# Kelvin-ywc/LPI

Measured on AMD Instinct MI355X. Metric: image-text pairs/sec fwd+bwd (ViT-B/16, bs256/GPU), higher is better.
Workload: dtype bf16; 1 GPU; BASELINE.json configs[2]: ViT-B/16 dual encoder bs=256/GPU prompt_depth=3 r=4 P=16, fwd+bwd incl. DecomposedPrompt grads + SGD step; global_batch=256, image=224x224, towers=lock step, GEMMs of one layer op grouped in one launch, parallelism=dp1, weights=synthetic (numpy Philox, CLIP-init scales), frozen

## Files before the change

include/lpi_hip.h:

```cpp
#ifndef LPI_HIP_H
#define LPI_HIP_H

#include <stdint.h>

#ifdef __cplusplus
extern "C" {
#endif

#define LPI_F32 0
#define LPI_BF16 1
#define LPI_F16 2

#define LPI_F32X3 4

#define LPI_EINVAL (-22)
#define LPI_ENOSYS (-38)

#define LPI_EPI_NONE 0
#define LPI_EPI_QUICKGELU 1
#define LPI_EPI_DQUICKGELU 2
#define LPI_EPI_LN 3
#define LPI_EPI_LN_QUICKGELU 4
#define LPI_EPI_RES_ROWSTATS 5

// ... 102 lines not shown
    const void* q; int ldq;
    const void* qkv; int ldqkv;
    const int32_t* idx;
    void* ctx; int ldctx;
    float* lse;
    const void* dctx; int lddctx;
    void* dq; int lddq;
    void* dqkv; int lddqkv;
    int causal;
    int shared_rows;
    float* shared_dkv;
} lpi_attn_pooled_desc;
int lpi_attn_pooled_fwd_pair(int dtype, const lpi_attn_pooled_desc* d , void* stream);
int lpi_attn_pooled_bwd_pair(int dtype, const lpi_attn_pooled_desc* d , void* stream);
int lpi_attn_pooled_fwd_desc(int dtype, const lpi_attn_pooled_desc* d, void* stream);
int lpi_attn_pooled_bwd_desc(int dtype, const lpi_attn_pooled_desc* d, void* stream);

int lpi_spool_attn_supported(int L, int H, int d);
int lpi_spool_attn_fwd(int w_dtype, int B, int L, int H, const void* q, int ldq, const void* Wqkv, int ldw, const void* WqkvT, int ldwt, const float* bqkv, const void* x, int ldx,
                       const float* mean, const float* rstd, const float* gamma, const float* beta, float* scratch, float* lse, void* ctx, int ldctx, void* stream);
int lpi_spool_attn_bwd(int B, int L, int H, const void* Wqkv , int ldw, const void* WqkvT , int ldwt, const void* x, int ldx, const float* mean,
                       const float* rstd, const float* gamma, float* scratch, const float* lse, const void* dctx, int lddctx, void* dq, int lddq, void* dh, int lddh,
                       void* stream);

int lpi_txt_embed_fwd_shared(int x_dtype, int B, int L, const int32_t* row_start, int shared_rows , int P, int d, const int64_t* ids,
                             const float* tok_emb, const float* pos, const float* ctx , void* x0, float* out_mean,
                             float* out_rstd, void* stream);
int lpi_attn_fwd_shared(int dtype, int B, int L, const int32_t* row_start, int shared_rows, int H, const void* qkv, int ldqkv, void* ctx, int ldctx,
                        float* lse, void* stream);
int lpi_attn_bwd_shared(int dtype, int B, int L, const int32_t* row_start, int shared_rows, int rows_needed, int H, const void* qkv, int ldqkv,
                        const void* ctx, int ldctx, const void* dctx, int lddctx, const float* lse, float* delta, void* dqkv, int lddqkv,
                        float* shared_dkv, void* stream);
int lpi_shared_kv_reduce(int dtype, int B, int shared_rows, int H, const float* partial, void* dqkv, int lddqkv, int accumulate, void* stream);
int lpi_layernorm_bwd_rows_varlen(int dy_dtype, int cast_dtype, int x_dtype, int B, int L, const int32_t* row_start, int row0, int P, int d,
                                  const void* dy, int lddy, const void* x, int ldx, const float* gamma, const float* mean, const float* rstd,
                                  float* dx, int lddx, void* dx_cast, int ldcast, int accumulate, void* stream);
int lpi_gather_batch_rows_varlen(int dtype, int B, int L, const int32_t* row_start, int row0, int P, int cols, const void* src, int ld_src,
                                 void* dst, int ld_dst, void* stream);
int lpi_rows_sum_over_batch_varlen(int dtype, int B, int L, const int32_t* row_start, int row0, int P, int d, const void* dx, float* out,
                                   int accumulate, void* stream);
int lpi_prompt_add_varlen(int x_dtype, int B, int L, const int32_t* row_start, int P, int d, void* x, const float* prompt_l, long prompt_bstride,
                          float* out_mean, float* out_rstd, void* stream);
int lpi_txt_embed_fwd_varlen(int x_dtype, int B, int L, const int32_t* row_start, int P, int d, const int64_t* ids, const float* tok_emb,
                             const float* pos, const float* ctx, long ctx_bstride, void* x0, float* out_mean, float* out_rstd, void* stream);

int lpi_prompt_cp_fwd(int Lyr, int P, int D, int r, const float* d1, const float* d2, const float* d3,
// ... 196 lines not shown
```

lpi_amd/_lib.py:

```python
from __future__ import annotations

import ctypes
import os
from ctypes import c_float, c_int, c_long, c_uint64, c_void_p

_HERE = os.path.dirname(os.path.abspath(__file__))
LIB_PATH = os.environ.get("LPI_LIB") or os.path.join(_HERE, "csrc", "liblpi_hip.so")

F32, BF16, F16 = 0, 1, 2
MX8 = 3
GEMM_K_128, GEMM_K_256, GEMM_K_256_TAIL, GEMM_K_256X128, GEMM_K_ROWS = 0, 1, 2, 3, 4
GEMM_K_MX8 = 5
F32X3 = 4
GEMM_K_X3 = 6
GEMM_K_MX8_256 = 7
EPI_NONE, EPI_QUICKGELU, EPI_DQUICKGELU, EPI_LN, EPI_LN_QUICKGELU, EPI_RES_ROWSTATS = 0, 1, 2, 3, 4, 5


class LpiError(RuntimeError):
    pass


class GemmDesc(ctypes.Structure):
    _fields_ = [("M", c_int), ("N", c_int), ("K", c_int), ("A", c_void_p), ("lda", c_int), ("B", c_void_p), ("ldb", c_int),
# ... 22 lines not shown
    "lpi_gemm_nt_mx8": [_I, _I, _I, _I, _P, _I, _P, _I, _P, _I, _P, _I, _P, _I, _P, _I, _P, _P, _I, _I, _F, _P],
    "lpi_gemm_mx8_256_ok": [_I, _I, _I],
    "lpi_gemm_nt_mx8_256": [_I, _I, _I, _I, _P, _I, _P, _I, _P, _I, _P, _I, _P, _I, _P, _I, _P, _P, _I, _I, _F, _P],
    "lpi_mx8_quantize": [_I, _I, _I, _P, _I, _P, _I, _P, _I, _P],
    "lpi_layernorm_mx8_fwd": [_I, _I, _I, _P, _I, _P, _P, _P, _I, _P, _I, _P, _P, _P],
    "lpi_layernorm_fwd": [_I, _I, _I, _I, _P, _I, _P, _P, _P, _I, _P, _P, _P],
    "lpi_layernorm_bwd": [_I, _I, _I, _I, _I, _P, _I, _P, _I, _P, _P, _P, _P, _I, _P, _I, _I, _P],
    "lpi_layernorm_fwd_pair": [_I, _I, _P, _P],
    "lpi_layernorm_bwd_pair": [_I, _I, _I, _P, _P],
    "lpi_layernorm_bwd_rows": [_I, _I, _I, _I, _I, _I, _I, _I, _P, _I, _P, _I, _P, _P, _P, _P, _I, _P, _I, _I, _P],
    "lpi_gather_batch_rows": [_I, _I, _I, _I, _I, _I, _P, _I, _P, _I, _P],
    "lpi_attn_fwd": [_I, _I, _I, _I, _P, _I, _P, _I, _P, _I, _P],
    "lpi_attn_bwd": [_I, _I, _I, _I, _P, _I, _P, _I, _P, _I, _P, _P, _P, _I, _I, _P],
    "lpi_attn_pooled_fwd": [_I, _I, _I, _I, _P, _I, _P, _I, _P, _P, _I, _P, _I, _P],
    "lpi_attn_pooled_bwd": [_I, _I, _I, _I, _P, _I, _P, _I, _P, _P, _I, _P, _P, _I, _P, _I, _I, _P],
    "lpi_attn_fwd_varlen": [_I, _I, _I, _P, _I, _P, _I, _P, _I, _P, _I, _P],
    "lpi_attn_bwd_varlen": [_I, _I, _I, _P, _I, _P, _I, _P, _I, _P, _I, _P, _P, _P, _I, _I, _P],
    "lpi_attn_fwd_pair": [_I, _P, _P],
    "lpi_attn_bwd_layout": [_I, _I, _I, _I, _I, _P, _I, _P, _I, _P, _I, _P, _P, _P, _I, _P, _P],
    "lpi_attn_fwd_one": [_I, _P, _P],
    "lpi_spool_attn_supported": [_I, _I, _I],
    "lpi_spool_attn_fwd": [_I, _I, _I, _I, _P, _I, _P, _I, _P, _I, _P, _P, _I, _P, _P, _P, _P, _P, _P, _P, _I, _P],
    "lpi_spool_attn_bwd": [_I, _I, _I, _P, _I, _P, _I, _P, _I, _P, _P, _P, _P, _P, _P, _I, _P, _I, _P, _I, _P],
    "lpi_attn_bwd_prefix": [_I, _I, _I, _P, _I, _I, _P, _I, _P, _I, _P, _I, _P, _P, _P, _I, _I, _P],
    "lpi_attn_pooled_fwd_varlen": [_I, _I, _I, _P, _I, _P, _I, _P, _I, _P, _P, _I, _P, _I, _P],
    "lpi_attn_pooled_bwd_varlen": [_I, _I, _I, _P, _I, _P, _I, _P, _I, _P, _P, _I, _P, _P, _I, _P, _I, _I, _P],
    "lpi_layernorm_bwd_rows_varlen": [_I, _I, _I, _I, _I, _P, _I, _I, _I, _P, _I, _P, _I, _P, _P, _P, _P, _I, _P, _I, _I, _P],
    "lpi_gather_batch_rows_varlen": [_I, _I, _I, _P, _I, _I, _I, _P, _I, _P, _I, _P],
    "lpi_rows_sum_over_batch_varlen": [_I, _I, _I, _P, _I, _I, _I, _P, _P, _I, _P],
    "lpi_prompt_add_varlen": [_I, _I, _I, _P, _I, _I, _P, _P, _L, _P, _P, _P],
    "lpi_txt_embed_fwd_varlen": [_I, _I, _I, _P, _I, _I, _P, _P, _P, _P, _L, _P, _P, _P, _P],
    "lpi_scatter_add_rows": [_I, _I, _I, _I, _P, _I, _P, _P, _I, _P],
    "lpi_prompt_cp_fwd": [_I, _I, _I, _I, _P, _P, _P, _F, _P, _P],
    "lpi_prompt_cp_bwd": [_I, _I, _I, _I, _P, _P, _P, _F, _P, _P, _P, _P, _I, _P, _P],
    "lpi_align_loss_fwd_bwd": [_I, _I, _I, _I, _P, _P, _F, _F, _P, _P, _P, _P],
    "lpi_nt_bxent_fwd_bwd": [_I, _I, _I, _P, _P, _F, _F, _P, _P, _I, _P, _P],
    "lpi_patchify": [_I, _I, _I, _I, _P, _P, _I, _P],
    "lpi_patchify_u8": [_I, _I, _I, _I, _P, _P, _P, _I, _P],
    "lpi_vis_assemble_fwd": [_I, _I, _I, _I, _I, _P, _I, _P, _P, _P, _L, _P, _P, _P, _P, _P, _P, _P, _P],
    "lpi_vis_assemble_bwd": [_I, _I, _I, _I, _I, _P, _P, _L, _P, _P, _P, _P, _P],
    "lpi_txt_embed_fwd": [_I, _I, _I, _I, _I, _P, _P, _P, _P, _L, _P, _P, _P, _P],
    "lpi_rows_sum_over_batch": [_I, _I, _I, _I, _I, _I, _P, _P, _I, _P],
    "lpi_prompt_add": [_I, _I, _I, _I, _I, _P, _P, _L, _P, _P, _P],
    "lpi_pool_ln_fwd": [_I, _I, _I, _I, _I, _P, _P, _P, _P, _P, _I, _P, _P, _P],
    "lpi_pool_ln_bwd": [_I, _I, _I, _I, _P, _I, _P, _P, _P, _P, _P, _P, _P, _P],
    "lpi_gather_rows": [_I, _I, _I, _I, _P, _P, _P, _P],
# ... 42 lines not shown
    "lpi_host_gather": [_P, _P, _I, _L, _I],
    "lpi_host_gather_v": [_P, _P, _P, _I, _I],
    "lpi_image_resample_workspace": [_I, _I, _P, _P],
    "lpi_image_resample_u8": [_I, _I, _P, _P, _L, _P, _L, _P, _P],
    "lpi_image_resample_workspace_f": [_I, _I, _I, _P, _P],
    "lpi_image_resample_u8_f": [_I, _I, _I, _P, _P, _L, _P, _L, _P, _P],
    "lpi_jpeg_info": [_P, _L, _P],
    "lpi_jpeg_decode_workspace": [_I, _P, _P, _P],
    "lpi_jpeg_decode_u8": [_I, _P, _P, _P, _L, _P, _P, _L, _P, _P, _L, _P],
    "lpi_jpeg_info_x": [_I, _P, _L, _P],
    "lpi_jpeg_decode_workspace_x": [_I, _I, _P, _P, _P],
    "lpi_jpeg_decode_u8_x": [_I, _I, _P, _P, _P, _L, _P, _P, _L, _P, _P, _L, _P],
    "lpi_bpe_create": [_P, _L],
    "lpi_bpe_destroy": [_P],
    "lpi_interact_workspace_floats": [_I, _I, _I, _I],
    "lpi_interact_fwd": [_I, _I, _I, _I, _I, _I, _P, _I, _P, _I, _P, _P, _P, _P, _P, _P, _P, _P, _P, _P, _F, _F, _P, _I, _P, _I, _P, _P],
    "lpi_interact_bwd": [_I, _I, _I, _I, _I, _I, _P, _I, _P, _I, _P, _P, _P, _P, _P, _P, _P, _P, _P, _P, _F, _F, _P, _I, _P, _I, _P, _I, _P, _I,
                         _P, _P, _P],
    "lpi_bpe_encode": [_P, _P, _P, _I],
    "lpi_bpe_tokenize": [_P, _P, _I, _I, _I, _P],
}
_RESTYPES = {"lpi_launch_count": c_uint64, "lpi_search_workspace": c_long, "lpi_bpe_create": c_void_p, "lpi_bpe_destroy": None}

EXPECTED_ABI = 618
VARIANT_OFFSET = 1000000

_lib = None


def load() -> ctypes.CDLL:
    global _lib
    if _lib is not None:
        return _lib
    import torch
    if not os.path.exists(LIB_PATH):
        raise LpiError(
            f"{LIB_PATH} not found: the MI355X HIP extension is not built. Run "
            f"`python -c 'import __graft_entry__ as g; g.build()'` or lpi_amd/csrc/build.sh. "
            f"There is no CPU fallback for the product path.")
    lib = ctypes.CDLL(LIB_PATH)
    for name, argtypes in SIGNATURES.items():
        try:
            fn = getattr(lib, name)
        except AttributeError as e:
            raise LpiError(f"{LIB_PATH} does not export {name}") from e
        fn.argtypes = argtypes
        fn.restype = _RESTYPES.get(name, c_int)
# ... 204 lines not shown
```

lpi_amd/csrc/api.hip:

```cpp
#include <atomic>
#include "common.h"

static std::atomic<uint64_t> g_launches{0};

extern "C" void lpi_count_launch() { g_launches.fetch_add(1, std::memory_order_relaxed); }
extern "C" uint64_t lpi_launch_count(void) { return g_launches.load(std::memory_order_relaxed); }
#ifndef LPI_ABI_VERSION
#define LPI_ABI_VERSION 618
#endif
#ifdef LPI_VARIANT_BUILD
extern "C" int lpi_version(void) { return LPI_ABI_VERSION + 1000000; }
#else
extern "C" int lpi_version(void) { return LPI_ABI_VERSION; }
#endif

int lpi_cu_count() {
    static std::atomic<int> cache[64];
    int dev = 0;
    if (hipGetDevice(&dev) != hipSuccess || dev < 0 || dev >= 64) dev = 0;
    int n = cache[dev].load(std::memory_order_relaxed);
    if (n == 0) {
        int v = 0;
        if (hipDeviceGetAttribute(&v, hipDeviceAttributeMultiprocessorCount, dev) != hipSuccess || v <= 0) v = 256;
        cache[dev].store(v, std::memory_order_relaxed);
        n = v;
    }
    return n;
}

static thread_local int t_last_gemm_kernel = -1;
void lpi_note_gemm_kernel(int which) { t_last_gemm_kernel = which; }
// ... 15 lines not shown
```

lpi_amd/csrc/attn_stream.hip:

```cpp
#include "common.h"
#include "../../include/lpi_hip.h"

namespace {

constexpr int HD = 64;
constexpr int HS = 16;
constexpr int NT = 512;
typedef __attribute__((ext_vector_type(2))) float f32x2;
typedef __attribute__((ext_vector_type(2))) _Float16 f16x2;

__device__ __forceinline__ float wave_sum(float v) {
#pragma unroll
    for (int o = 32; o > 0; o >>= 1) v += __shfl_xor(v, o);
    return v;
}
__device__ __forceinline__ float wave_max(float v) {
#pragma unroll
    for (int o = 32; o > 0; o >>= 1) v = fmaxf(v, __shfl_xor(v, o));
    return v;
}


template <typename T>
__global__ __launch_bounds__(256) void headw_t_kernel(int B, int H, int d, const T* __restrict__ in, int ldin, const T* __restrict__ WT, int ldwt, int col0, float scale,
// ... 375 lines not shown
                    if (l < L) *reinterpret_cast<uint2*>(orow + (jt + u) * 16) = make_uint2(pack2_t<bf16_t>(acc[0], acc[1]), pack2_t<bf16_t>(acc[2], acc[3]));
                }
            }
        }
    }
    {
        constexpr int NJ = KS / 4;
        f32x4 acc[NJ];
#pragma unroll
        for (int t = 0; t < NJ; ++t) acc[t] = f32x4{0.f, 0.f, 0.f, 0.f};
        weighted_row_sums_mfma<NJ, NJ>(acc, A.x + row0 * A.ldx, A.ldx, L, Lp, d, wt, xt);
        const int h = lane & 15, g = lane >> 4;
        if (h < H) {
            const float zm = zmu[h];
#pragma unroll
            for (int t = 0; t < NJ; ++t) {
                const int j = 16 * (wave + 8 * t) + 4 * g;
                if (j < d) *reinterpret_cast<f32x4*>(A.dqt + ((size_t)b * H + h) * d + j) = *reinterpret_cast<const f32x4*>(A.gamma + j) * (acc[t] - zm);
            }
        }
    }
}

size_t spool_lds(int L, int d, bool bwd) {
    const size_t Lp = (size_t)((L + 15) & ~15), rb = (size_t)d * 2 + 16;
    const size_t Lp32 = (Lp + 31) & ~(size_t)31, wt = HS * Lp32 * 2, xt = 32 * ((size_t)d * 2 + XT_PAD);
    if (!bwd) return HS * rb + Lp * HS * 4 + 2 * Lp * 4 + 2 * HS * 4 + wt + xt;
    return std::max(std::max(2 * HS * rb, (size_t)d * W2B), xt) + 2 * Lp * HS * 4 + Lp * 64 + 2 * Lp * 4 + 3 * HS * 4 + wt;
}

bool spool_ok(int L, int H, int d) { return H >= 1 && H <= HS && d == HD * H && d % 32 == 0 && d <= 2 * NT && L >= 1 && L <= 288 && spool_lds(L, d, true) <= 160 * 1024; }

template <bool BWD>
int spool_launch(const SpoolArgs& A, hipStream_t s) {
    const int KS = A.d / 32, NH = (A.H + 3) & ~3;
    const size_t lds = spool_lds(A.L, A.d, BWD);
#define SP(K, N)                                                                                                                   \
    if (KS == K && NH == N) {                                                                                                      \
        static LdsOnce once;                                                                                                       \
        const void* fn = BWD ? (const void*)spool_bwd_kernel<K, N> : (const void*)spool_fwd_kernel<K, N>;                          \
        if (int e = lpi_ensure_lds(once, fn, 160 * 1024)) return e;                                                                \
        if (BWD) LPI_LAUNCH((spool_bwd_kernel<K, N>), dim3(A.B), dim3(NT), lds, s, A);                                              \
        else LPI_LAUNCH((spool_fwd_kernel<K, N>), dim3(A.B), dim3(NT), lds, s, A);                                                  \
        LPI_CHECK_LAST();                                                                                                          \
        return 0;                                                                                                                  \
    }
    SP(24, 12) SP(32, 16) SP(4, 4) SP(8, 4) SP(16, 8)
#undef SP
    return LPI_ENOSYS;
}

template <typename T>
int headw_t(int B, int H, int d, const void* in, int ldin, const void* WT, int ldwt, int col0, float scale, float* out, hipStream_t s) {
    LPI_LAUNCH((headw_t_kernel<T>), dim3(H, (B + 15) / 16), dim3(256), 0, s, B, H, d, (const T*)in, ldin, (const T*)WT, ldwt, col0, scale, out);
// ... 30 lines not shown
    return w_dtype == LPI_BF16 ? headw_n<bf16_t, bf16_t>(B, H, d, hbar, Wqkv, ldw, 2 * d, bqkv, 1.0f, ctx, ldctx, s)
                               : headw_n<f16_t, f16_t>(B, H, d, hbar, Wqkv, ldw, 2 * d, bqkv, 1.0f, ctx, ldctx, s);
}

extern "C" int lpi_spool_attn_bwd(int B, int L, int H, const void* Wqkv, int ldw, const void* WqkvT, int ldwt, const void* x, int ldx, const float* mean,
                                  const float* rstd, const float* gamma, float* scratch, const float* lse, const void* dctx, int lddctx, void* dq, int lddq, void* dh,
                                  int lddh, void* stream) {
    const int d = HD * H;
    if (!Wqkv || !WqkvT || !x || !mean || !rstd || !gamma || !scratch || !lse || !dctx || !dq || !dh || B <= 0) return LPI_EINVAL;
    if (!spool_ok(L, H, d) || ldw < d || ldwt < 3 * d || ldx < d || lddctx < d || lddq < d || lddh < d || ((ldx | ldw | ldwt | lddctx) & 7) || (lddh & 3) ||
        (((uintptr_t)x | (uintptr_t)Wqkv | (uintptr_t)WqkvT | (uintptr_t)dctx) & 15) || ((uintptr_t)dh & 7) ||
        (((uintptr_t)scratch | (uintptr_t)gamma) & 15))
        return LPI_EINVAL;
    hipStream_t s = (hipStream_t)stream;
    const size_t n = (size_t)B * H * d;
    float* qt = scratch;
    float* dhbar = scratch + 2 * n;
    float* dqt = scratch + 3 * n;
    if (int e = headw_t<bf16_t>(B, H, d, dctx, lddctx, WqkvT, ldwt, 2 * d, 1.0f, dhbar, s)) return e;
    SpoolArgs A{B, L, H, d, (const f16_t*)x, ldx, mean, rstd, gamma, nullptr, qt, nullptr, const_cast<float*>(lse), dhbar, (bf16_t*)dh, lddh, dqt};
    if (int e = spool_launch<true>(A, s)) return e;
    return headw_n<bf16_t, bf16_t>(B, H, d, dqt, Wqkv, ldw, d, nullptr, 0.125f, dq, lddq, s);
}
```

lpi_amd/engine.py:

```python
from __future__ import annotations

import math
from dataclasses import dataclass
from typing import Optional

import numpy as np
import torch

from . import _lib
from ._lib import BF16, EPI_DQUICKGELU, EPI_LN, EPI_LN_QUICKGELU, EPI_NONE, EPI_QUICKGELU, EPI_RES_ROWSTATS, F16, F32, F32X3, call
from .synth import ClipConfig

import ctypes
import os as _os

_DT = {"f32": F32, "fp32": F32, "float32": F32, "bf16": BF16, "bfloat16": BF16, "f16": F16, "fp16": F16, "float16": F16, "half": F16}


def _grad_dtype(dt: int) -> int:
    return F32 if dt == F32 else BF16
_TORCH_DT = {F32: torch.float32, BF16: torch.bfloat16, F16: torch.float16}


PIXEL_NORMS = {"imagenet": (None, None),
               "clip": ((0.48145466, 0.4578275, 0.40821073), (0.26862954, 0.26130258, 0.27577711))}


@dataclass(frozen=True)
class EngineOptions:
    residual_f16: bool = True
    ln_fold: int = 2
    rowstats: int = 2
    rowstat_guard: bool = True
    pooled_last: bool = True
    stream_pool: bool = True
    l0_prompt_rows: bool = True
    qkv_grouped: bool = False
    pixel_norm: object = "imagenet"
    mx8_forward: bool = False
    mx8_tile256: bool = True
    gemm_bf16x3: bool = False

    def __post_init__(self):
        if self.ln_fold not in (0, 1, 2) or self.rowstats not in (0, 1, 2):
            raise ValueError("ln_fold and rowstats are 0, 1 or 2")
        if not isinstance(self.pixel_norm, str):
            try:
                mean, std = self.pixel_norm
                pair = (tuple(float(v) for v in mean), tuple(float(v) for v in std))
            except (TypeError, ValueError):
                raise ValueError(f"pixel_norm is 'imagenet', 'clip' or a (mean, std) pair, not {self.pixel_norm!r}") from None
            if len(pair[0]) != 3 or len(pair[1]) != 3:
                raise ValueError("pixel_norm: a (mean, std) pair holds three values each")
            object.__setattr__(self, "pixel_norm", pair)
        elif self.pixel_norm not in PIXEL_NORMS:
            raise ValueError(f"pixel_norm is 'imagenet', 'clip' or a (mean, std) pair, not {self.pixel_norm!r}")

    def check_dtype(self, dtype: str):
# ... 476 lines not shown
        Lreal, L = L, max(L, cap or L)
        Mp = _pad(B * L, 256)
        Bp = _pad(B)
        T, TX, TG = _TORCH_DT[self.dt], _TORCH_DT[self.xdt], _TORCH_DT[self.gdt]
        TU = TG if self.dt == F16 else T
        dev = self.device
        z = lambda *s, dtype=torch.float32: torch.zeros(*s, dtype=dtype, device=dev)
        keep = nl if train else 1
        ws = {
            "B": B, "L": L, "Mp": Mp, "Lcap": L,
            "x": [z(Mp, d, dtype=TX) for _ in range(nl + 1 if train else 2)],
            "xmid": [z(Mp, d, dtype=TX) for _ in range(keep)],
            "qkv": [z(Mp, 3 * d, dtype=T) for _ in range(keep)],
            "ctx": [z(Mp, d, dtype=T) for _ in range(keep)],
            "lse": [z(B + 1, H, L) for _ in range(keep)],
            "u": [z(Mp, 4 * d, dtype=TU) for _ in range(keep)] if train else [None],
            "lnblk": [z(2, 3 * Mp + 4 * d) for _ in range(nl)],
            "h": z(Mp, d, dtype=T),
            "g": z(Mp, 4 * d, dtype=T),
            "rstat": z(2 * max(d // 128, 1), Mp),
            "Bp": Bp, "c_xmid": z(Bp, d), "c_h": z(Bp, d, dtype=T), "c_g": z(Bp, 4 * d, dtype=T),
            "c_u": z(Bp, 4 * d, dtype=TU) if train else None, "c_xout": z(Bp, d), "c_stat": z(2, Bp),
            "c_q": z(Bp, d, dtype=T), "c_ctx": z(Bp, d, dtype=T), "c_lse": z(B * H), "c_xin": z(Bp, d), "c_stat1": z(2, Bp),
            "sp_scratch": z(4 * B * H * d) if self._stream_pool_shape(L) else None, "sp_lse": z(B * H),
        }
        if train:
            ws.update({
                "dx": z(Mp, d) if self.dt == F32 else None,
                "dh": z(Mp, d, dtype=TG), "dctx": z(Mp, d, dtype=TG), "dqkv": z(Mp, 3 * d, dtype=TG),
                "delta": z(B + 1, H, L),
                "dxT": z(Mp, d, dtype=TG) if self.dt != F32 else None,
                "c_dx": z(Bp, d), "c_dxT": z(Bp, d, dtype=TG) if self.dt != F32 else None, "c_dh": z(Bp, d, dtype=TG),
                "c_dctx": z(Bp, d, dtype=TG), "c_dq": z(Bp, d, dtype=TG),
                "p_dqkv": z(_pad(B * 32, 256), 3 * d, dtype=TG), "p_dh": z(_pad(B * 32, 256), d, dtype=TG),
                "du": None, "c_du": None,
            })
        if train:
            ws["du"], ws["c_du"] = ws["g"].view(TG), ws["c_g"].view(TG)
        if self.mx8 and not train:
            u8 = lambda *s: torch.zeros(*s, dtype=torch.uint8, device=dev)
            ws["mx"] = {"h": u8(Mp, d), "hs": u8(Mp, d // 32), "ctx": u8(Mp, d), "ctxs": u8(Mp, d // 32), "g": u8(Mp, 4 * d), "gs": u8(Mp, 4 * d // 32)}
        ws["stat"] = [(b[0, :Mp], b[0, Mp:2 * Mp], b[1, :Mp], b[1, Mp:2 * Mp]) for b in ws["lnblk"]]
        ws["ln_ld"] = Mp
        for i, blk in enumerate(self.blocks):
            if "qkv_ln" in blk:
                c1 = blk["qkv_ln"].c1
                if i == nl - 1 and POOLED_LAST:
# ... 137 lines not shown
        dxT = ws["dxT"] if dt != F32 else dx
        P = prompts.shape[-2] if prompts is not None else 0
        pre = ws.get("pre", 0)
        Bq, Lq, rsq = (1, pre, None) if pre else (B, L, rs)
        self._check_depth(prompts, depth)
        for i in reversed(range(len(self.blocks))):
            blk = self.blocks[i]
            lt = "last" if i == len(self.blocks) - 1 else f"r{len(self.blocks) - 1 - i}"
            x_in, xmid, qkv, ctx, lse, u, st = ws["x"][i], ws["xmid"][i], ws["qkv"][i], ws["ctx"][i], ws["lse"][i], ws["u"][i], ws["stat"][i]
            if i == len(self.blocks) - 1 and not POOLED_LAST:
                call("lpi_zero", dxT, dxT.numel() * dxT.element_size(), s)
                call("lpi_scatter_rows", dt, B, Lx, d, ws["c_dx"], pidx, dx, None if dt == F32 else dxT, s)
            if i == len(self.blocks) - 1 and POOLED_LAST:
                Bp, cst = ws["Bp"], ws["c_stat"]
                c_dx = ws["c_dx"]
                c_dxT = ws["c_dxT"] if dt != F32 else c_dx
                yield GemmReq(f"{lt}.cdproj", mdt, c_dxT, blk["proj"].wt, ws["c_du"], Bp, 4 * d, d, epi=EPI_DQUICKGELU, aux=ws["c_u"], m_real=B)
                yield GemmReq(f"{lt}.cdfc", mdt, ws["c_du"], blk["fc"].wt, ws["c_dh"], Bp, d, 4 * d, m_real=B)
                yield RowReq(f"{lt}.cdln2", [_lib.row_job(_lib.ROWOP_LN_BWD, B=B, d=d, dt_a=dt, dt_b=dt, a=ws["c_dh"], ld_a=d, b=ws["c_xmid"], ld_b=d,
                                                          gamma=blk["ln_2.w"], mean_in=cst[0], rstd_in=cst[1], out=c_dx, out2=None if dt == F32 else c_dxT,
                                                          ld_c=d, flag=1)])
                wqt = blk["qkv"].wt
                yield GemmReq(f"{lt}.cdout", mdt, c_dxT, blk["out"].wt, ws["c_dctx"], Bp, d, d, m_real=B)
                if rs is None and not pre and ws.get("sp_scratch") is not None and self._stream_pool_shape(L):
                    yield SoloReq(f"{lt}.pdattn", lambda: call("lpi_spool_attn_bwd", B, L, H, blk["qkv_wb"], d, blk["qkv"].wt, 3 * d, x_in, d, st[0], st[1], blk["ln_1.w"],
                                                               ws["sp_scratch"], ws["sp_lse"], ws["c_dctx"], d, ws["c_dq"], d, dh, d, _stream()))
                    yield SoloReq(f"{lt}.dkv")
                else:
                    yield PoolAttnReq(f"{lt}.pdattn", adt, True, B=B, L=L, row_start=rs, H=H, q=ws["c_q"], ldq=d, qkv=qkv, ldqkv=3 * d, idx=pool_idx,
                                      dctx=ws["c_dctx"], lddctx=d, lse=ws["c_lse"], dq=ws["c_dq"], lddq=d, dqkv=dqkv, lddqkv=3 * d, causal=int(sp.causal),
                                      shared_rows=pre, shared_dkv=ws.get("shared_dkv") if pre else None)
                    yield GemmReq(f"{lt}.dkv", mdt, dqkv[:, d:], wqt[:, d:], dh, Mp, d, 2 * d, m_real=M)
                yield GemmReq(f"{lt}.cdq", mdt, ws["c_dq"], wqt[:, :d], ws["c_dh"], Bp, d, d, m_real=B)
                yield RowReq(f"{lt}.sadd1", [_lib.row_job(_lib.ROWOP_SCATTER_ADD, B=B, L=Lx, d=d, dt_a=dt, a=ws["c_dh"], ld_a=d, idx=pidx, out=dh, ld_c=d)])
                yield LnReq(f"{lt}.dln1", "bwd", (dt, dt, xdt), M, d, dh, d, x_in, d, blk["ln_1.w"], st[0], st[1], dx, d,
                            None if dt == F32 else dxT, d, 0)
                yield RowReq(f"{lt}.sadd2", [_lib.row_job(_lib.ROWOP_SCATTER_ADD, B=B, L=Lx, d=d, dt_a=dt, a=c_dxT, ld_a=d, idx=pidx, out=dxT, ld_c=d)])
                if prompts is not None and dprompts is not None and 0 < i < depth:
                    yield RowsSumReq(f"{lt}.psum", dt, Bq, Lq, rsq, 1, P, d, dxT, dprompts[i], acc)
                continue
            if not (i == len(self.blocks) - 1 and POOLED_LAST):
                du = ws["du"]
                yield GemmReq(f"{lt}.dproj", mdt, dxT, blk["proj"].wt, du, Mp, 4 * d, d, epi=EPI_DQUICKGELU, aux=u, m_real=M)
                yield GemmReq(f"{lt}.dfc", mdt, du, blk["fc"].wt, dh, Mp, d, 4 * d, m_real=M)
                yield LnReq(f"{lt}.dln2", "bwd", (dt, dt, xdt), M, d, dh, d, xmid, d, blk["ln_2.w"], st[2], st[3], dx, d,
                            None if dt == F32 else dxT, d, 1)
            yield GemmReq(f"{lt}.dout", mdt, dxT, blk["out"].wt, dctx, Mp, d, d, m_real=M)
            l0_rows = i == 0 and L0_PROMPT_ROWS and prompts is not None and 0 < P <= 32 and len(self.blocks) > 1
            if pre:
                call("lpi_attn_bwd_shared", adt, B, L, rs, pre, (1 + P) if l0_rows else L, H, qkv, 3 * d, ctx, d, dctx, d, lse, ws["delta"], dqkv, 3 * d,
                     ws["shared_dkv"], s)
            elif blk["grouped"]:
                hs_, vs_, chs_ = self.qkv_lay
                lay = (ctypes.c_int32 * 6)(hs_, vs_, hs_, vs_, chs_, chs_)
                call("lpi_attn_bwd_layout", adt, B, L, (1 + P) if l0_rows else L, H, qkv, 3 * d, ctx, d, dctx, d, lse, ws["delta"], dqkv, 3 * d,
                     ctypes.cast(lay, ctypes.c_void_p), s)
# ... 599 lines not shown
```

Before: 11710 pairs/s.

## Fuse LN1 backward into streaming pooled-attention backward for last layer

Adds a streaming pooled-attention backward kernel that computes the LayerNorm-1 backward for every non-pooled row in place and writes bf16 dx directly. Only the pooled row's dy goes to a small fp32 buffer. A tiny follow-up kernel finishes the LN backward for that pooled row, adding the cdq and residual contributions. This removes the full-size dh intermediate, the scatter-add and the separate M x d LayerNorm backward pass over all tokens. In exchange the fused kernel carries more LDS and register pressure, and it rounds dy to bf16 inside the kernel.

```diff
diff --git a/include/lpi_hip.h b/include/lpi_hip.h
--- a/include/lpi_hip.h
+++ b/include/lpi_hip.h
@@ -148,6 +148,11 @@
 int lpi_spool_attn_bwd(int B, int L, int H, const void* Wqkv , int ldw, const void* WqkvT , int ldwt, const void* x, int ldx, const float* mean,
                        const float* rstd, const float* gamma, float* scratch, const float* lse, const void* dctx, int lddctx, void* dq, int lddq, void* dh, int lddh,
                        void* stream);
+int lpi_spool_attn_bwd_ln1(int B, int L, int H, const void* Wqkv , int ldw, const void* WqkvT , int ldwt, const void* x, int ldx, const float* mean,
+                           const float* rstd, const float* gamma, const float* beta, float* scratch, const float* lse, const void* dctx, int lddctx, void* dq, int lddq,
+                           const int* pidx, void* dxs, int lddxs, float* dpool, void* stream);
+int lpi_spool_pool_rows(int B, int L, int d, const int* pidx, const float* dpool, const void* c_dh, int ldcdh, const void* c_dx, int ldcdx, const void* x, int ldx,
+                        const float* mean, const float* rstd, const float* gamma, void* dxs, int lddxs, void* stream);
 
 int lpi_txt_embed_fwd_shared(int x_dtype, int B, int L, const int32_t* row_start, int shared_rows , int P, int d, const int64_t* ids,
                              const float* tok_emb, const float* pos, const float* ctx , void* x0, float* out_mean,
diff --git a/lpi_amd/_lib.py b/lpi_amd/_lib.py
--- a/lpi_amd/_lib.py
+++ b/lpi_amd/_lib.py
@@ -68,6 +68,8 @@
     "lpi_spool_attn_supported": [_I, _I, _I],
     "lpi_spool_attn_fwd": [_I, _I, _I, _I, _P, _I, _P, _I, _P, _I, _P, _P, _I, _P, _P, _P, _P, _P, _P, _P, _I, _P],
     "lpi_spool_attn_bwd": [_I, _I, _I, _P, _I, _P, _I, _P, _I, _P, _P, _P, _P, _P, _P, _I, _P, _I, _P, _I, _P],
+    "lpi_spool_attn_bwd_ln1": [_I, _I, _I, _P, _I, _P, _I, _P, _I, _P, _P, _P, _P, _P, _P, _P, _I, _P, _I, _P, _P, _I, _P, _P],
+    "lpi_spool_pool_rows": [_I, _I, _I, _P, _P, _P, _I, _P, _I, _P, _I, _P, _P, _P, _P, _I, _P],
     "lpi_attn_bwd_prefix": [_I, _I, _I, _P, _I, _I, _P, _I, _P, _I, _P, _I, _P, _P, _P, _I, _I, _P],
     "lpi_attn_pooled_fwd_varlen": [_I, _I, _I, _P, _I, _P, _I, _P, _I, _P, _P, _I, _P, _I, _P],
     "lpi_attn_pooled_bwd_varlen": [_I, _I, _I, _P, _I, _P, _I, _P, _I, _P, _P, _I, _P, _P, _I, _P, _I, _I, _P],
@@ -156,7 +158,7 @@
 }
 _RESTYPES = {"lpi_launch_count": c_uint64, "lpi_search_workspace": c_long, "lpi_bpe_create": c_void_p, "lpi_bpe_destroy": None}
 
-EXPECTED_ABI = 618
+EXPECTED_ABI = 619
 VARIANT_OFFSET = 1000000
 
 _lib = None
diff --git a/lpi_amd/csrc/api.hip b/lpi_amd/csrc/api.hip
--- a/lpi_amd/csrc/api.hip
+++ b/lpi_amd/csrc/api.hip
@@ -6,7 +6,7 @@
 extern "C" void lpi_count_launch() { g_launches.fetch_add(1, std::memory_order_relaxed); }
 extern "C" uint64_t lpi_launch_count(void) { return g_launches.load(std::memory_order_relaxed); }
 #ifndef LPI_ABI_VERSION
-#define LPI_ABI_VERSION 618
+#define LPI_ABI_VERSION 619
 #endif
 #ifdef LPI_VARIANT_BUILD
 extern "C" int lpi_version(void) { return LPI_ABI_VERSION + 1000000; }
diff --git a/lpi_amd/csrc/attn_stream.hip b/lpi_amd/csrc/attn_stream.hip
--- a/lpi_amd/csrc/attn_stream.hip
+++ b/lpi_amd/csrc/attn_stream.hip
@@ -421,6 +421,329 @@
     }
 }
 
+struct Spool1Args {
+    int B, L, H, d;
+    const f16_t* x; int ldx;
+    const float* mean; const float* rstd;
+    const float* gamma; const float* beta;
+    const float* qt; const float* hbar; const float* lse; const float* dhbar;
+    float* dqt;
+    const int* pidx;
+    bf16_t* dxs; int lddxs;
+    float* dpool;
+};
+
+constexpr int PART_BYTES = 8 * 2 * 2 * 16 * 16 * 4;
+
+template <int KS>
+__global__ __launch_bounds__(NT) void spool_bwd1_kernel(Spool1Args A) {
+    static_assert(KS % 4 == 0, "d is a multiple of 128");
+    constexpr int NJ = KS / 4, NKW = (KS + 7) / 8;
+    extern __shared__ __attribute__((aligned(16))) char smem[];
+    const int b = blockIdx.x, tid = threadIdx.x, lane = tid & 63, wave = tid >> 6, g = lane >> 4, r16 = lane & 15;
+    constexpr int d = 32 * KS, rsx = d * 2 + XT_PAD, cpr = d / 8;
+    const int L = A.L, H = A.H, Lp32 = (L + 31) & ~31, rb = grow_bytes(d);
+    char* xt = smem;
+    char* img0 = smem;
+    char* img1 = smem + HS * rb;
+    float* part = reinterpret_cast<float*>(smem + 32 * rsx);
+    char* PD = reinterpret_cast<char*>(part) + PART_BYTES;
+    char* wt = PD + 32 * 64;
+    float* red = reinterpret_cast<float*>(wt + 2 * HS * 32 * 2);
+    float* gam = red + 8 * 32 * 2;
+    float* mu_l = gam + d;
+    float* rs_l = mu_l + Lp32;
+    float* cg = rs_l + Lp32;
+    float* cgd = cg + HS;
+    float* dl = cgd + HS;
+    float* lse_s = dl + HS;
+    float* zmu = lse_s + HS;
+    const size_t row0 = (size_t)b * L;
+    const float* qtb = A.qt + (size_t)b * H * d;
+    const float* dhb = A.dhbar + (size_t)b * H * d;
+    const float* hbb = A.hbar + (size_t)b * H * d;
+    const int pl = A.pidx ? min(max(A.pidx[b], 0), L - 1) : 0;
+    stage_row_stats(mu_l, rs_l, A.mean, A.rstd, row0, L, Lp32);
+    for (int j = tid; j < d; j += NT) gam[j] = A.gamma[j];
+    if (tid < HS) lse_s[tid] = tid < H ? A.lse[(size_t)b * H + tid] : 0.f;
+    for (int h = wave; h < HS; h += NT / 64) {
+        float s = 0.f;
+        if (h < H)
+            for (int j = lane; j < d; j += 64) {
+                const float gm = A.gamma[j], dv = dhb[(size_t)h * d + j];
+                s += (hbb[(size_t)h * d + j] - A.beta[j]) * (gm != 0.f ? (float)(f16_t)(gm * dv) / gm : dv);
+            }
+        s = wave_sum(s);
+        if (lane == 0) dl[h] = s;
+    }
+    Chunk w2[NJ];
+#pragma unroll
+    for (int t = 0; t < NJ; ++t) {
+        const int j = 16 * (wave * NJ + t) + r16, hb = (g & 1) * 8;
+        const float* src = (g < 2 ? dhb : qtb) + j;
+        float v[8];
+#pragma unroll
+        for (int q = 0; q < 8; ++q) v[q] = hb + q < H ? src[(size_t)(hb + q) * d] : 0.f;
+        w2[t].u = make_uint4(pack2_t<f16_t>(v[0], v[1]), pack2_t<f16_t>(v[2], v[3]), pack2_t<f16_t>(v[4], v[5]), pack2_t<f16_t>(v[6], v[7]));
+        __builtin_amdgcn_sched_barrier(0);
+    }
+    fill_gamma_image(img0, cg, qtb, A.gamma, H, d);
+    fill_gamma_image(img1, cgd, dhb, A.gamma, H, d);
+    Chunk ia[NKW], ib[NKW];
+#pragma unroll
+    for (int c = 0; c < NKW; ++c) {
+        const int ks = wave + 8 * c;
+        ia[c].u = ib[c].u = make_uint4(0, 0, 0, 0);
+        if (ks < KS) {
+            ia[c].u = *reinterpret_cast<const uint4*>(img0 + r16 * rb + (g + 4 * ks) * 16);
+            ib[c].u = *reinterpret_cast<const uint4*>(img1 + r16 * rb + (g + 4 * ks) * 16);
+        }
+    }
+    f32x4 accq[NJ];
+#pragma unroll
+    for (int t = 0; t < NJ; ++t) accq[t] = f32x4{0.f, 0.f, 0.f, 0.f};
+    float zm = 0.f, spd = 0.f, sw = 0.f;
+    const f16_t* xs = A.x + row0 * A.ldx;
+    uint4 stg[NJ];
+    auto load_tile = [&](int l0) {
+#pragma unroll
+        for (int u = 0; u < NJ; ++u) {
+            const int c = tid + u * NT;
+            stg[u] = make_uint4(0, 0, 0, 0);
+            if (c < 32 * cpr) stg[u] = *reinterpret_cast<const uint4*>(xs + (size_t)min(l0 + c / cpr, L - 1) * A.ldx + (c % cpr) * 8);
+        }
+    };
+    load_tile(0);
+    for (int l0 = 0; l0 < Lp32; l0 += 32) {
+        __syncthreads();
+#pragma unroll
+        for (int u = 0; u < NJ; ++u) {
+            const int c = tid + u * NT;
+            if (c < 32 * cpr) *reinterpret_cast<uint4*>(xt + (c / cpr) * rsx + (c % cpr) * 16) = stg[u];
+        }
+        __syncthreads();
+        if (l0 + 32 < Lp32) load_tile(l0 + 32);
+#pragma unroll
+        for (int hf = 0; hf < 2; ++hf) {
+            f32x4 a0 = f32x4{0.f, 0.f, 0.f, 0.f}, a1 = f32x4{0.f, 0.f, 0.f, 0.f};
+#pragma unroll
+            for (int c = 0; c < NKW; ++c) {
+                const int ks = wave + 8 * c;
+                Chunk xb;
+                xb.u = make_uint4(0, 0, 0, 0);
+                if (ks < KS) xb.u = *reinterpret_cast<const uint4*>(xt + (hf * 16 + r16) * rsx + (g + 4 * ks) * 16);
+                mma_chunk<f16_t>(a0, ia[c], xb);
+                mma_chunk<f16_t>(a1, ib[c], xb);
+            }
+            float* pp = part + ((wave * 2 + hf) * 2 * 16 + r16) * 16 + 4 * g;
+            *reinterpret_cast<f32x4*>(pp) = a0;
+            *reinterpret_cast<f32x4*>(pp + 16 * 16) = a1;
+        }
+        __syncthreads();
+        {
+            const int row = tid >> 4, h = tid & 15, l = l0 + row;
+            float a0 = 0.f, a1 = 0.f;
+#pragma unroll
+            for (int w = 0; w < 8; ++w) {
+                const float* pp = part + ((w * 2 + (row >> 4)) * 2 * 16 + (row & 15)) * 16 + h;
+                a0 += pp[0];
+                a1 += pp[16 * 16];
+            }
+            const float mu = mu_l[l], rs = rs_l[l];
+            float p = 0.f, ds = 0.f;
+            if (l < L && h < H) {
+                p = __expf(rs * (a0 - mu * cg[h]) - lse_s[h]);
+                const float dp = rs * (a1 - mu * cgd[h]), pw = (float)(f16_t)(p * rs) / rs;
+                ds = pw * (dp - dl[h]);
+                spd += pw * dp;
+                sw += pw;
+            }
+            const f16_t e = (f16_t)(ds * rs), e2 = (f16_t)(ds * rs - (float)e);
+            zm += ((float)e + (float)e2) * mu;
+            *reinterpret_cast<f16_t*>(PD + row * 64 + h * 2) = (f16_t)p;
+            *reinterpret_cast<f16_t*>(PD + row * 64 + 32 + h * 2) = (f16_t)ds;
+            *reinterpret_cast<f16_t*>(wt + (h * 32 + row) * 2) = e;
+            *reinterpret_cast<f16_t*>(wt + (HS * 32 + h * 32 + row) * 2) = e2;
+        }
+        __syncthreads();
+        auto g_tile = [&](int row, int t, const Chunk& pd, float mu, float rs, f32x4& dy, f32x4& gv, f32x4& xh) {
+            const int col = 16 * (wave * NJ + t) + 4 * g;
+            f32x4 acc = f32x4{0.f, 0.f, 0.f, 0.f};
+            mma_chunk<f16_t>(acc, w2[t], pd);
+            const f32x4 xv = Elem<f16_t>::ld4(reinterpret_cast<const f16_t*>(xt + row * rsx) + col);
+            const uint32_t r01 = pack2_t<bf16_t>(acc[0], acc[1]), r23 = pack2_t<bf16_t>(acc[2], acc[3]);
+            dy = f32x4{__uint_as_float(r01 << 16), __uint_as_float(r01 & 0xFFFF0000u), __uint_as_float(r23 << 16), __uint_as_float(r23 & 0xFFFF0000u)};
+            gv = dy * *reinterpret_cast<const f32x4*>(gam + col);
+            xh = (xv - mu) * rs;
+        };
+#pragma unroll
+        for (int hf = 0; hf < 2; ++hf) {
+            const int row = hf * 16 + r16;
+            Chunk pd;
+            pd.u = *reinterpret_cast<const uint4*>(PD + row * 64 + g * 16);
+            const float mu = mu_l[l0 + row], rs = rs_l[l0 + row];
+            float s1 = 0.f, s2 = 0.f;
+#pragma unroll
+            for (int t = 0; t < NJ; ++t) {
+                f32x4 dy, gv, xh;
+                g_tile(row, t, pd, mu, rs, dy, gv, xh);
+#pragma unroll
+                for (int i = 0; i < 4; ++i) {
+                    s1 += gv[i];
+                    s2 += gv[i] * xh[i];
+                }
+            }
+            s1 += __shfl_xor(s1, 16);
+            s2 += __shfl_xor(s2, 16);
+            s1 += __shfl_xor(s1, 32);
+            s2 += __shfl_xor(s2, 32);
+            if (g == 0) *reinterpret_cast<f32x2*>(red + (wave * 32 + row) * 2) = f32x2{s1, s2};
+        }
+        {
+            Chunk wb, wb2;
+            const uint2 lo = *reinterpret_cast<const uint2*>(wt + (r16 * 32 + 4 * g) * 2), hi = *reinterpret_cast<const uint2*>(wt + (r16 * 32 + 16 + 4 * g) * 2);
+            wb.u = make_uint4(lo.x, lo.y, hi.x, hi.y);
+            const uint2 lob = *reinterpret_cast<const uint2*>(wt + (HS * 32 + r16 * 32 + 4 * g) * 2), hib = *reinterpret_cast<const uint2*>(wt + (HS * 32 + r16 * 32 + 16 + 4 * g) * 2);
+            wb2.u = make_uint4(lob.x, lob.y, hib.x, hib.y);
+            const char* tp = xt + (4 * g + (r16 >> 2)) * rsx + (r16 & 3) * 8;
+#pragma unroll
+            for (int t = 0; t < NJ; ++t) {
+                const int jt = wave + 8 * t;
+                const short4s tlo = __builtin_amdgcn_ds_read_tr16_b64_v4i16((__attribute__((address_space(3))) short4s*)(tp + jt * 32));
+                const short4s thi = __builtin_amdgcn_ds_read_tr16_b64_v4i16((__attribute__((address_space(3))) short4s*)(tp + 16 * rsx + jt * 32));
+                const uint2 lo2 = __builtin_bit_cast(uint2, tlo), hi2 = __builtin_bit_cast(uint2, thi);
+                Chunk xa;
+                xa.u = make_uint4(lo2.x, lo2.y, hi2.x, hi2.y);
+                mma_chunk<f16_t>(accq[t], xa, wb);
+                mma_chunk<f16_t>(accq[t], xa, wb2);
+            }
+        }
+        __syncthreads();
+#pragma unroll
+        for (int hf = 0; hf < 2; ++hf) {
+            const int row = hf * 16 + r16, l = l0 + row;
+            float c1 = 0.f, c2 = 0.f;
+#pragma unroll
+            for (int w = 0; w < 8; ++w) {
+                const f32x2 q = *reinterpret_cast<const f32x2*>(red + (w * 32 + row) * 2);
+                c1 += q[0];
+                c2 += q[1];
+            }
+            c1 /= (float)d;
+            c2 /= (float)d;
+            const float mu = mu_l[l], rs = rs_l[l];
+            const bool pooled = l == pl;
+            Chunk pd;
+            pd.u = *reinterpret_cast<const uint4*>(PD + row * 64 + g * 16);
+            bf16_t* orow = A.dxs + (row0 + l) * A.lddxs + 4 * g;
+            float* prow = A.dpool + (size_t)b * d + 4 * g;
+#pragma unroll
+            for (int t = 0; t < NJ; ++t) {
+                f32x4 dy, gv, xh;
+                g_tile(row, t, pd, mu, rs, dy, gv, xh);
+                if (l < L) {
+                    if (pooled) {
+                        *reinterpret_cast<f32x4*>(prow + 16 * (wave * NJ + t)) = dy;
+                    } else {
+                        const f32x4 o = (gv - c1 - xh * c2) * rs;
+                        *reinterpret_cast<uint2*>(orow + 16 * (wave * NJ + t)) = make_uint2(pack2_t<bf16_t>(o[0], o[1]), pack2_t<bf16_t>(o[2], o[3]));
+                    }
+                }
+            }
+        }
+    }
+    __syncthreads();
+    part[tid] = zm;
+    part[NT + tid] = spd;
+    part[2 * NT + tid] = sw;
+    __syncthreads();
+    if (tid < HS) {
+        float s = 0.f, sp = 0.f, ws = 0.f;
+        for (int r = 0; r < 32; ++r) {
+            s += part[r * 16 + tid];
+            sp += part[NT + r * 16 + tid];
+            ws += part[2 * NT + r * 16 + tid];
+        }
+        zmu[tid] = s;
+        dl[tid] -= ws > 0.f ? sp / ws : 0.f;
+    }
+    __syncthreads();
+    if (r16 < H) {
+        const float z = zmu[r16], off = dl[r16];
+#pragma unroll
+        for (int t = 0; t < NJ; ++t) {
+            const int j = 16 * (wave + 8 * t) + 4 * g;
+            const f32x4 hb4 = *reinterpret_cast<const f32x4*>(A.hbar + ((size_t)b * H + r16) * d + j) - *reinterpret_cast<const f32x4*>(A.beta + j);
+            *reinterpret_cast<f32x4*>(A.dqt + ((size_t)b * H + r16) * d + j) = *reinterpret_cast<const f32x4*>(gam + j) * (accq[t] - z) + hb4 * off;
+        }
+    }
+}
+
+__global__ __launch_bounds__(256) void spool_pool_rows_kernel(int B, int L, int d, const int* __restrict__ pidx, const float* __restrict__ dpool, const bf16_t* __restrict__ cdh,
+                                                              int ldcdh, const bf16_t* __restrict__ cdx, int ldcdx, const f16_t* __restrict__ x, int ldx,
+                                                              const float* __restrict__ mean, const float* __restrict__ rstd, const float* __restrict__ gamma,
+                                                              bf16_t* __restrict__ dxs, int lddxs) {
+    const int b = blockIdx.x * 4 + (threadIdx.x >> 6), lane = threadIdx.x & 63;
+    if (b >= B) return;
+    const size_t row = (size_t)b * L + (pidx ? min(max(pidx[b], 0), L - 1) : 0);
+    const float mu = mean[row], rs = rstd[row];
+    const f16_t* xr = x + row * ldx;
+    f32x4 gj[4], xh[4];
+    float s1 = 0.f, s2 = 0.f;
+#pragma unroll
+    for (int u = 0; u < 4; ++u) {
+        const int j = 4 * lane + 256 * u;
+        gj[u] = xh[u] = f32x4{0.f, 0.f, 0.f, 0.f};
+        if (j < d) {
+            const f32x4 dy = *reinterpret_cast<const f32x4*>(dpool + (size_t)b * d + j) + Elem<bf16_t>::ld4(cdh + (size_t)b * ldcdh + j);
+            const uint32_t r01 = pack2_t<bf16_t>(dy[0], dy[1]), r23 = pack2_t<bf16_t>(dy[2], dy[3]);
+            gj[u] = f32x4{__uint_as_float(r01 << 16), __uint_as_float(r01 & 0xFFFF0000u), __uint_as_float(r23 << 16), __uint_as_float(r23 & 0xFFFF0000u)} *
+                    *reinterpret_cast<const f32x4*>(gamma + j);
+            xh[u] = (Elem<f16_t>::ld4(xr + j) - mu) * rs;
+        }
+    }
+#pragma unroll
+    for (int u = 0; u < 4; ++u)
+#pragma unroll
+        for (int i = 0; i < 4; ++i) {
+            s1 += gj[u][i];
+            s2 += gj[u][i] * xh[u][i];
+        }
+    const float c1 = wave_sum(s1) / (float)d, c2 = wave_sum(s2) / (float)d;
+#pragma unroll
+    for (int u = 0; u < 4; ++u) {
+        const int j = 4 * lane + 256 * u;
+        if (j < d) {
+            const f32x4 o = (gj[u] - c1 - xh[u] * c2) * rs;
+            const uint32_t r01 = pack2_t<bf16_t>(o[0], o[1]), r23 = pack2_t<bf16_t>(o[2], o[3]);
+            const f32x4 ob = f32x4{__uint_as_float(r01 << 16), __uint_as_float(r01 & 0xFFFF0000u), __uint_as_float(r23 << 16), __uint_as_float(r23 & 0xFFFF0000u)} +
+                             Elem<bf16_t>::ld4(cdx + (size_t)b * ldcdx + j);
+            *reinterpret_cast<uint2*>(dxs + row * lddxs + j) = make_uint2(pack2_t<bf16_t>(ob[0], ob[1]), pack2_t<bf16_t>(ob[2], ob[3]));
+        }
+    }
+}
+
+size_t spool1_lds(int L, int d) {
+    const size_t Lp32 = (size_t)((L + 31) & ~31);
+    return 32 * ((size_t)d * 2 + XT_PAD) + PART_BYTES + 32 * 64 + 2 * HS * 32 * 2 + 8 * 32 * 2 * 4 + (size_t)d * 4 + 2 * Lp32 * 4 + 5 * HS * 4;
+}
+
+int spool1_launch(const Spool1Args& A, hipStream_t s) {
+    const int KS = A.d / 32;
+    const size_t lds = spool1_lds(A.L, A.d);
+#define SP1(K)                                                                               \
+    if (KS == K) {                                                                           \
+        static LdsOnce once;                                                                 \
+        if (int e = lpi_ensure_lds(once, (const void*)spool_bwd1_kernel<K>, 160 * 1024)) return e; \
+        LPI_LAUNCH((spool_bwd1_kernel<K>), dim3(A.B), dim3(NT), lds, s, A);                  \
+        LPI_CHECK_LAST();                                                                    \
+        return 0;                                                                            \
+    }
+    SP1(24) SP1(32) SP1(4) SP1(8) SP1(16)
+#undef SP1
+    return LPI_ENOSYS;
+}
+
 size_t spool_lds(int L, int d, bool bwd) {
     const size_t Lp = (size_t)((L + 15) & ~15), rb = (size_t)d * 2 + 16;
     const size_t Lp32 = (Lp + 31) & ~(size_t)31, wt = HS * Lp32 * 2, xt = 32 * ((size_t)d * 2 + XT_PAD);
@@ -428,7 +751,9 @@
     return std::max(std::max(2 * HS * rb, (size_t)d * W2B), xt) + 2 * Lp * HS * 4 + Lp * 64 + 2 * Lp * 4 + 3 * HS * 4 + wt;
 }
 
-bool spool_ok(int L, int H, int d) { return H >= 1 && H <= HS && d == HD * H && d % 32 == 0 && d <= 2 * NT && L >= 1 && L <= 288 && spool_lds(L, d, true) <= 160 * 1024; }
+bool spool_ok(int L, int H, int d) {
+    return H >= 1 && H <= HS && d == HD * H && d % 32 == 0 && d <= 2 * NT && L >= 1 && L <= 288 && spool_lds(L, d, true) <= 160 * 1024 && spool1_lds(L, d) <= 160 * 1024;
+}
 
 template <bool BWD>
 int spool_launch(const SpoolArgs& A, hipStream_t s) {
@@ -505,3 +830,33 @@
     if (int e = spool_launch<true>(A, s)) return e;
     return headw_n<bf16_t, bf16_t>(B, H, d, dqt, Wqkv, ldw, d, nullptr, 0.125f, dq, lddq, s);
 }
+
+extern "C" int lpi_spool_attn_bwd_ln1(int B, int L, int H, const void* Wqkv, int ldw, const void* WqkvT, int ldwt, const void* x, int ldx, const float* mean,
+                                      const float* rstd, const float* gamma, const float* beta, float* scratch, const float* lse, const void* dctx, int lddctx, void* dq,
+                                      int lddq, const int* pidx, void* dxs, int lddxs, float* dpool, void* stream) {
+    const int d = HD * H;
+    if (!Wqkv || !WqkvT || !x || !mean || !rstd || !gamma || !beta || !scratch || !lse || !dctx || !dq || !dxs || !dpool || B <= 0) return LPI_EINVAL;
+    if (!spool_ok(L, H, d) || d % 128 || ldw < d || ldwt < 3 * d || ldx < d || lddctx < d || lddq < d || lddxs < d || ((ldx | ldw | ldwt | lddctx) & 7) || (lddxs & 3) ||
+        (((uintptr_t)x | (uintptr_t)Wqkv | (uintptr_t)WqkvT | (uintptr_t)dctx) & 15) || ((uintptr_t)dxs & 7) ||
+        (((uintptr_t)scratch | (uintptr_t)gamma | (uintptr_t)beta | (uintptr_t)dpool) & 15))
+        return LPI_EINVAL;
+    hipStream_t s = (hipStream_t)stream;
+    const size_t n = (size_t)B * H * d;
+    float* dhbar = scratch + 2 * n;
+    float* dqt = scratch + 3 * n;
+    if (int e = headw_t<bf16_t>(B, H, d, dctx, lddctx, WqkvT, ldwt, 2 * d, 1.0f, dhbar, s)) return e;
+    Spool1Args A{B, L, H, d, (const f16_t*)x, ldx, mean, rstd, gamma, beta, scratch, scratch + n, lse, dhbar, dqt, pidx, (bf16_t*)dxs, lddxs, dpool};
+    if (int e = spool1_launch(A, s)) return e;
+    return headw_n<bf16_t, bf16_t>(B, H, d, dqt, Wqkv, ldw, d, nullptr, 0.125f, dq, lddq, s);
+}
+
+extern "C" int lpi_spool_pool_rows(int B, int L, int d, const int* pidx, const float* dpool, const void* c_dh, int ldcdh, const void* c_dx, int ldcdx, const void* x, int ldx,
+                                   const float* mean, const float* rstd, const float* gamma, void* dxs, int lddxs, void* stream) {
+    if (!dpool || !c_dh || !c_dx || !x || !mean || !rstd || !gamma || !dxs || B <= 0 || L <= 0 || d <= 0 || d > 1024 || (d & 3) || ldcdh < d || ldcdx < d || ldx < d || lddxs < d ||
+        ((ldcdh | ldcdx | ldx | lddxs) & 3) || (((uintptr_t)c_dh | (uintptr_t)c_dx | (uintptr_t)x | (uintptr_t)dxs) & 7) || (((uintptr_t)dpool | (uintptr_t)gamma) & 15))
+        return LPI_EINVAL;
+    LPI_LAUNCH(spool_pool_rows_kernel, dim3((B + 3) / 4), dim3(256), 0, (hipStream_t)stream, B, L, d, pidx, dpool, (const bf16_t*)c_dh, ldcdh, (const bf16_t*)c_dx, ldcdx,
+               (const f16_t*)x, ldx, mean, rstd, gamma, (bf16_t*)dxs, lddxs);
+    LPI_CHECK_LAST();
+    return 0;
+}
diff --git a/lpi_amd/engine.py b/lpi_amd/engine.py
--- a/lpi_amd/engine.py
+++ b/lpi_amd/engine.py
@@ -34,6 +34,7 @@
     rowstat_guard: bool = True
     pooled_last: bool = True
     stream_pool: bool = True
+    spool_ln1: bool = True
     l0_prompt_rows: bool = True
     qkv_grouped: bool = False
     pixel_norm: object = "imagenet"
@@ -556,7 +557,7 @@
             "Bp": Bp, "c_xmid": z(Bp, d), "c_h": z(Bp, d, dtype=T), "c_g": z(Bp, 4 * d, dtype=T),
             "c_u": z(Bp, 4 * d, dtype=TU) if train else None, "c_xout": z(Bp, d), "c_stat": z(2, Bp),
             "c_q": z(Bp, d, dtype=T), "c_ctx": z(Bp, d, dtype=T), "c_lse": z(B * H), "c_xin": z(Bp, d), "c_stat1": z(2, Bp),
-            "sp_scratch": z(4 * B * H * d) if self._stream_pool_shape(L) else None, "sp_lse": z(B * H),
+            "sp_scratch": z(4 * B * H * d + B * d) if self._stream_pool_shape(L) else None, "sp_lse": z(B * H),
         }
         if train:
             ws.update({
@@ -740,7 +741,15 @@
                                                           ld_c=d, flag=1)])
                 wqt = blk["qkv"].wt
                 yield GemmReq(f"{lt}.cdout", mdt, c_dxT, blk["out"].wt, ws["c_dctx"], Bp, d, d, m_real=B)
-                if rs is None and not pre and ws.get("sp_scratch") is not None and self._stream_pool_shape(L):
+                spool = rs is None and not pre and ws.get("sp_scratch") is not None and self._stream_pool_shape(L)
+                fused = bool(spool and self.opt.spool_ln1 and dt == BF16 and d % 128 == 0)
+                dpool = ws["sp_scratch"][4 * B * H * d:4 * B * H * d + B * d] if fused else None
+                if fused:
+                    yield SoloReq(f"{lt}.pdattn", lambda: call("lpi_spool_attn_bwd_ln1", B, L, H, blk["qkv_wb"], d, blk["qkv"].wt, 3 * d, x_in, d, st[0], st[1], blk["ln_1.w"],
+                                                               blk["ln_1.b"], ws["sp_scratch"], ws["sp_lse"], ws["c_dctx"], d, ws["c_dq"], d, pidx, dxT, d,
+                                                               dpool, _stream()))
+                    yield SoloReq(f"{lt}.dkv")
+                elif spool:
                     yield SoloReq(f"{lt}.pdattn", lambda: call("lpi_spool_attn_bwd", B, L, H, blk["qkv_wb"], d, blk["qkv"].wt, 3 * d, x_in, d, st[0], st[1], blk["ln_1.w"],
                                                                ws["sp_scratch"], ws["sp_lse"], ws["c_dctx"], d, ws["c_dq"], d, dh, d, _stream()))
                     yield SoloReq(f"{lt}.dkv")
@@ -750,6 +759,14 @@
                                       shared_rows=pre, shared_dkv=ws.get("shared_dkv") if pre else None)
                     yield GemmReq(f"{lt}.dkv", mdt, dqkv[:, d:], wqt[:, d:], dh, Mp, d, 2 * d, m_real=M)
                 yield GemmReq(f"{lt}.cdq", mdt, ws["c_dq"], wqt[:, :d], ws["c_dh"], Bp, d, d, m_real=B)
+                if fused:
+                    yield SoloReq(f"{lt}.sadd1")
+                    yield SoloReq(f"{lt}.dln1")
+                    yield SoloReq(f"{lt}.sadd2", lambda: call("lpi_spool_pool_rows", B, L, d, pidx, dpool, ws["c_dh"], d, c_dxT, d, x_in, d, st[0], st[1],
+                                                              blk["ln_1.w"], dxT, d, _stream()))
+                    if prompts is not None and dprompts is not None and 0 < i < depth:
+                        yield RowsSumReq(f"{lt}.psum", dt, Bq, Lq, rsq, 1, P, d, dxT, dprompts[i], acc)
+                    continue
                 yield RowReq(f"{lt}.sadd1", [_lib.row_job(_lib.ROWOP_SCATTER_ADD, B=B, L=Lx, d=d, dt_a=dt, a=ws["c_dh"], ld_a=d, idx=pidx, out=dh, ld_c=d)])
                 yield LnReq(f"{lt}.dln1", "bwd", (dt, dt, xdt), M, d, dh, d, x_in, d, blk["ln_1.w"], st[0], st[1], dx, d,
                             None if dt == F32 else dxT, d, 0)
```

Result: no change. 11730 pairs/s, median of 6 (+0.1%).
